# maniacs-ops/ringpop-go

Hardware: AMD Instinct MI355X
Metric: simulated member-rounds/sec at 64k members (higher is better)
Workload: dtype u32; 1 GPU; config3_cascade: 65536 members, 655 killed at r=10; rounds 5-592 timed (steady state, kill, suspect wave; faulty wave from r>=35 in window); members=65536, live_member_rounds=38153303, parallelism=1 GPU

## Files before the change

ringpop-go_amd/csrc/swimsim_engine.hip:

```cpp
#include "swimsim_kernels.hip"
#include "swimsim_xchg.hip"
#include "swimsim_census.hip"
#include "swimsim_route.hip"
#include "swimsim_forward.hip"
#include "swimsim_ringcs.hip"

#include <hipcub/hipcub.hpp>
#include <rccl/rccl.h>

#include <algorithm>
#include <cmath>
#include <condition_variable>
#include <cstdarg>
#include <cstdio>
#include <cstring>
#include <memory>
#include <mutex>
#include <string>
#include <thread>
#include <vector>

#include "../../include/swimsim.h"

using namespace swimdev;
// ... 305 lines not shown
    std::vector<hipEvent_t> round_ev;
    std::vector<float> round_ms;
    std::vector<uint32_t> wslot_h;
    std::vector<uint8_t> wused;
    std::vector<uint32_t> wcs;
    std::vector<uint32_t> wcs_ev;
    std::vector<uint4 *> wev_h;
    std::vector<unsigned long long *> wevt_h;
    uint4 *wout = nullptr;
    uint32_t *winfo = nullptr;
    uint32_t *cn_slab = nullptr, *cn_part = nullptr, *cn_nlp = nullptr, *cn_ticket = nullptr, *cn_cols = nullptr,
             *cn_res = nullptr;
    size_t cn_cap = 0;
    hipEvent_t cn_ev[2] = {nullptr, nullptr};
    uint32_t *tr_cols = nullptr, *tr_buf = nullptr, *tr_part = nullptr, *tr_nlp = nullptr, *tr_state = nullptr;
    uint32_t tr_n = 0, tr_cap = 0;
    size_t tr_bytes[5] = {0, 0, 0, 0, 0};
    struct RouteTable {
        uint32_t R;
        uint32_t *hm;
        unsigned long long *pts;
    };
    std::vector<RouteTable> rt_tabs;
    uint8_t *rt_bytes = nullptr;
    uint64_t *rt_off = nullptr;
    uint32_t *rt_kh = nullptr, *rt_p0 = nullptr, *rt_rows = nullptr, *rt_cnt = nullptr;
    int32_t *rt_base = nullptr, *rt_own = nullptr;
    uint32_t *rt_srv = nullptr;
    int32_t *rt_nbase = nullptr;
    size_t rt_srv_cap = 0, rt_nbase_cap = 0;
    unsigned long long *rt_exc = nullptr, *rt_exc2 = nullptr, *rt_uniq = nullptr, *rt_cur = nullptr;
    void *rt_cub = nullptr;
    size_t rt_bytes_cap = 0, rt_keys_cap = 0, rt_rows_cap = 0, rt_own_cap = 0, rt_exc_cap = 0, rt_cub_bytes = 0;
    std::vector<uint64_t> rt_rel;
    hipEvent_t rt_ev[2] = {nullptr, nullptr};
    unsigned long long *rc_key = nullptr;
    uint32_t *rc_cnt = nullptr, *rc_rep = nullptr, *rc_dif = nullptr, *rc_hl = nullptr, *rc_csr = nullptr, *rc_out = nullptr;
    size_t rc_cap = 0;
    bool rc_lds = false;
    double rc_split[3] = {0, 0, 0};
    int32_t *fw_own = nullptr, *fw_handler = nullptr, *fw_holder = nullptr, *fw_next = nullptr;
    uint32_t *fw_ent = nullptr, *fw_key = nullptr, *fw_bins = nullptr;
    uint8_t *fw_outcome = nullptr, *fw_hops = nullptr;
    size_t fw_own_cap = 0, fw_req_cap = 0, fw_ent_cap = 0, fw_bins_cap = 0;
    double fw_split[3] = {0, 0, 0};
    int csr_mode = 1;
    CsrSet csr, csr2;
    size_t csr_sbw_words = 0;
    uint32_t csr_ecap = 4096, csr_rcap = 1024, csr_KP = 0;
    uint64_t csr_launches = 0;
    uint32_t csr_side_min = 4097;
    int fault_inject = 0;
    int defer_test = 0;
    int cs_defer = 1;
    uint32_t rounds_left = 0;
    uint32_t round_deferred = 0;
    bool cs_carried = false;
    int resp_echo = 1;
    bool cs_defer_log = false;
    uint64_t cs_skipped_rounds = 0, cs_carried_rows = 0, cs_forced = 0, cs_units_base[3] = {0, 0, 0};
    bool colx_stale = false;
    std::string err;

    int fail(int code, const char *fmt, ...) {
        char buf[512];
        va_list ap;
        va_start(ap, fmt);
        vsnprintf(buf, sizeof buf, fmt, ap);
        va_end(ap);
        err = buf;
        return code;
    }
};

#define HIPCHK(h, x)                                                                             \
    do {                                                                                         \
        hipError_t e_ = (x);                                                                     \
        if (e_ != hipSuccess) return (h)->fail(SWIMSIM_EHIP, "%s: %s", #x, hipGetErrorString(e_)); \
    } while (0)

namespace {

template <typename T>
int dalloc(swimsim *h, T **p, size_t count, const char *what) {
    void *q = nullptr;
    size_t bytes = std::max<size_t>(count * sizeof(T), 16);
    hipError_t e = hipMalloc(&q, bytes);
    if (e != hipSuccess) return h->fail(SWIMSIM_ENOMEM, "hipMalloc(%s, %zu bytes): %s", what, bytes, hipGetErrorString(e));
    h->allocs.push_back(q);
    h->alloc_bytes += bytes;
    *p = (T *)q;
    return 0;
}

template <typename T>
void dfree(swimsim *h, T **p, size_t bytes) {
    if (!*p) return;
    auto it = std::find(h->allocs.begin(), h->allocs.end(), (void *)*p);
    if (it != h->allocs.end()) h->allocs.erase(it);
    hipFree(*p);
    h->alloc_bytes -= bytes;
    *p = nullptr;
}

hipEvent_t take_event(swimsim *h) {
    if (!h->evpool.empty()) {
        hipEvent_t e = h->evpool.back();
        h->evpool.pop_back();
        return e;
    }
    hipEvent_t e;
    hipEventCreate(&e);
    return e;
}

struct Scope {
    swimsim *h;
    int fam;
    hipStream_t st;
    hipEvent_t a{}, b{};
    bool on;
    Scope(swimsim *h_, int f, hipStream_t st_ = nullptr)
        : h(h_), fam(f), st(st_ ? st_ : h_->s), on(h_->timing && ((h_->timing_mask >> f) & 1u)) {
        if (on) {
            a = take_event(h);
            hipEventRecord(a, st);
        }
    }
    ~Scope() {
        if (on) {
            b = take_event(h);
            hipEventRecord(b, st);
            h->pending.push_back(Timed{fam, a, b});
        }
    }
};

void drain_timing(swimsim *h) {
    if (h->pending.empty()) return;
    hipStreamSynchronize(h->s);
    for (auto &t : h->pending) {
        float ms = 0;
        hipEventElapsedTime(&ms, t.a, t.b);
        h->fam_ms[t.fam] += ms;
        h->fam_n[t.fam]++;
        h->evpool.push_back(t.a);
        h->evpool.push_back(t.b);
    }
    h->pending.clear();
}

constexpr uint32_t SWIM_WAVE_BLOCK = 256;
constexpr uint32_t kWavesPerBlock = SWIM_WAVE_BLOCK / 64;
inline uint32_t blocks_for_waves(uint32_t waves) { return waves ? (waves + kWavesPerBlock - 1) / kWavesPerBlock : 1; }
inline uint32_t blocks_for_threads(uint32_t n) { return n ? (n + 255) / 256 : 1; }
inline uint32_t rep_slots(uint32_t nl) { uint32_t s = 1024; while (s < 2 * nl) s <<= 1; return s; }

constexpr uint32_t kMaxEcap = 1u << 24;

int build_tail_table(swimsim *h, uint32_t ecap) {
    if (ecap > kMaxEcap)
        return h->fail(SWIMSIM_ERANGE, "incarnation step %u beyond the checksum tables (at most 2^24 steps of the period)",
                       ecap - 1);
    std::vector<uint32_t> t((size_t)ecap * 4 * 8, 0u);
    uint32_t max_tl = 0, min_tl = 0xFFFFFFFFu;
    for (uint32_t e = 0; e < ecap; e++) {
        char digits[32];
        snprintf(digits, sizeof digits, "%lld", (long long)(h->t0 + (int64_t)e * h->period));
        for (uint32_t s = 0; s < 4; s++) {
            char buf[64];
            int n = snprintf(buf, sizeof buf, "%s%s;", kStatus[s], digits);
            if (n > 24) return h->fail(SWIMSIM_EINVAL, "incarnation %s too long for the checksum tail table", digits);
            uint8_t bytes[24] = {0};
            memcpy(bytes, buf, (size_t)n);
            uint32_t *dst = &t[((size_t)e * 4 + s) * 8];
            for (int w = 0; w < 6; w++)
                dst[w] = (uint32_t)bytes[4 * w] | ((uint32_t)bytes[4 * w + 1] << 8) | ((uint32_t)bytes[4 * w + 2] << 16) |
                         ((uint32_t)bytes[4 * w + 3] << 24);
            dst[6] = (uint32_t)n;
            max_tl = std::max(max_tl, (uint32_t)n);
            min_tl = std::min(min_tl, (uint32_t)n);
        }
    }
    std::vector<uint32_t> rt((size_t)ecap * 4 * 8, 0u);
    const uint32_t q = h->W / 4, r = h->W % 4;
    for (size_t i = 0; i < (size_t)ecap * 4; i++) {
        uint8_t bytes[32] = {0};
        const uint32_t n = t[i * 8 + 6];
        memcpy(bytes + r, &t[i * 8], n);
        for (int w = 0; w < 7; w++)
            rt[i * 8 + w] = (uint32_t)bytes[4 * w] | ((uint32_t)bytes[4 * w + 1] << 8) | ((uint32_t)bytes[4 * w + 2] << 16) |
                            ((uint32_t)bytes[4 * w + 3] << 24);
        const uint32_t L = h->W + n;
        const uint8_t *tb = (const uint8_t *)&t[i * 8];
        rt[i * 8 + 7] = (uint32_t)tb[n - 4] | ((uint32_t)tb[n - 3] << 8) | ((uint32_t)tb[n - 2] << 16) |
                        ((uint32_t)tb[n - 1] << 24);
        if (r + n > 27) return h->fail(SWIMSIM_EINVAL, "record tail too long for the checksum tail table");
        rt[i * 8 + 6] |= L << 24;
    }
    (void)q;
    std::vector<uint32_t> rt8((size_t)ecap * 8 * 8, 0u);
    for (size_t e = 0; e < ecap; e++)
        for (int s = 0; s < 4; s++) memcpy(&rt8[(e * 8 + s) * 8], &rt[(e * 4 + s) * 8], 32);
    uint32_t *dev = nullptr, *rdev = nullptr, *r8dev = nullptr;
    if (int rc = dalloc(h, &dev, t.size(), "tail table")) return rc;
    if (int rc = dalloc(h, &rdev, rt.size(), "record tail table")) return rc;
    if (int rc = dalloc(h, &r8dev, rt8.size(), "record tail table by member word")) return rc;
    HIPCHK(h, hipMemcpy(dev, t.data(), t.size() * 4, hipMemcpyHostToDevice));
    HIPCHK(h, hipMemcpy(rdev, rt.data(), rt.size() * 4, hipMemcpyHostToDevice));
    HIPCHK(h, hipMemcpy(r8dev, rt8.data(), rt8.size() * 4, hipMemcpyHostToDevice));
    h->d.tailw = dev;
    h->d.rtail = rdev;
    h->d.rtail8 = r8dev;
    {
        uint32_t d0 = t[6] - 6, nthr = 0;
        for (int k = 0; k < 8; k++) h->d.dig_thr[k] = 0xFFFFFFFFu;
        uint32_t prev = d0;
        for (uint32_t e = 1; e < ecap; e++) {
            const uint32_t de = t[((size_t)e * 4) * 8 + 6] - 6;
            if (de != prev) {
                if (de != prev + 1 || nthr == 8) return h->fail(SWIMSIM_EINVAL, "incarnation digit count changes too often");
                h->d.dig_thr[nthr++] = e;
                prev = de;
            }
        }
        h->d.dig_d0 = d0;
    }
    h->ecap = ecap;
    h->d.ecap = ecap;
    h->max_tl = max_tl;
    h->d.max_tail = max_tl;
    h->d.min_tail = min_tl;
    h->fast_cs = (h->W == 19 && h->W + max_tl <= 40);
    return 0;
}

hipError_t stream_sync(swimsim *h) {
    if (!h->sync_spin || !h->ev_rt) return hipStreamSynchronize(h->s);
    const hipError_t prior = hipPeekAtLastError();
    hipError_t e = hipEventRecord(h->ev_rt, h->s);
    if (e != hipSuccess) return e;
    while ((e = hipEventQuery(h->ev_rt)) == hipErrorNotReady) {
    }
    (void)hipGetLastError();
    return prior != hipSuccess ? prior : e;
}

int check_err(swimsim *h) {
    uint32_t e = 0;
    HIPCHK(h, hipMemcpyAsync(&e, h->d.err, 4, hipMemcpyDeviceToHost, h->s));
    HIPCHK(h, stream_sync(h));
    if (!e) return 0;
    hipMemsetAsync(h->d.err, 0, 4, h->s);
    if (e & E_POOL) return h->fail(SWIMSIM_ECAPACITY, "message pool overflow (raise message_pool_bytes)");
    if (e & E_DENSE) return h->fail(SWIMSIM_ECAPACITY, "dense snapshot pool overflow");
    if (e & E_ECAP) return h->fail(SWIMSIM_ECAPACITY, "incarnation beyond the checksum table");
    if (e & E_SHORT) return h->fail(SWIMSIM_EINVAL, "checksum string of <= 24 bytes is not supported");
    if (e & E_ITER) return h->fail(SWIMSIM_EINVAL, "iterator found no pingable member despite a positive count");
    return h->fail(SWIMSIM_EINVAL, "dissemination count mismatch (internal error %u)", e);
}

int read_counters(swimsim *h, uint64_t *out ) {
    std::vector<uint64_t> c((size_t)CTR_SHARDS * CTR_STRIDE);
    HIPCHK(h, hipMemcpyAsync(c.data(), h->d.ctr, c.size() * 8, hipMemcpyDeviceToHost, h->s));
    HIPCHK(h, stream_sync(h));
    for (int i = 0; i < CTR_STRIDE; i++) {
        uint64_t t = 0;
        for (int k = 0; k < CTR_SHARDS; k++) t += c[(size_t)k * CTR_STRIDE + i];
        out[i] = t;
    }
    return 0;
}

int build_inbox(swimsim *h, uint32_t nlocal, uint32_t n) {
    Scope sc(h, F_SORT);
    h->inbox_n = n;
    if (n > nlocal)
        hipLaunchKernelGGL(k_inbox_count, dim3(blocks_for_threads(n - nlocal)), dim3(256), 0, h->s, h->d, h->keys, nlocal,
                           n, h->counts, h->kslot);
    h->scan_gen = h->scan_gen % 0x1FFFFFu + 1u;
    hipLaunchKernelGGL(k_inbox_scan, dim3((h->NL + 1023) / 1024), dim3(1024), 0, h->s, h->d, h->counts, h->offs,
                       h->ulist, h->scan_agg, h->scan_gen);
    hipLaunchKernelGGL(k_inbox_place, dim3(blocks_for_threads(n)), dim3(256), 0, h->s, h->d, h->keys, n, h->offs,
                       h->kslot, h->vals_in, h->run_of);
    return 0;
}

inline uint32_t owner_host(const swimsim *h, uint32_t o) {
    uint32_t r = 0;
    while (r + 1 < h->G && o >= h->shard_lo[r + 1]) r++;
    return r;
}

XArgs xargs(swimsim *h) {
    XArgs x{};
    x.sdesc = h->sdesc; x.sdesc2 = h->sdesc2; x.rdesc = h->rdesc; x.rdesc2 = h->rdesc2; x.snapdesc = h->snapdesc;
    x.hdesc = h->hdesc;
    x.sI = h->sI; x.sC = h->sC; x.sI2 = h->sI2; x.sC2 = h->sC2;
    x.hsics = h->hsics;
    x.need = h->need;
    x.keys = h->keys; x.npairs = h->npairs; x.keycap = h->keycap;
    x.needlist = h->needlist; x.needcnt = h->needcnt; x.needcap = h->needcap;
    x.sS = h->sS; x.sS2 = h->sS2; x.rcs = h->rcs;
    x.csreq = h->csreq; x.csreqcnt = h->csreqcnt; x.csreqcap = h->keycap;
    return x;
}
// ... 2414 lines not shown
```

ringpop-go_amd/csrc/swimsim_kernels.hip:

```cpp
#include "swimsim_kernels.h"

namespace swimdev {

#define SWIM_DPP(old, src, ctrl, rm) ((uint32_t)__builtin_amdgcn_update_dpp((int)(old), (int)(src), (ctrl), (rm), 0xf, false))
template <typename Op>
__device__ __forceinline__ uint32_t dpp_scan(uint32_t x, uint32_t id, Op op) {
    x = op(x, SWIM_DPP(id, x, 0x111, 0xf));
    x = op(x, SWIM_DPP(id, x, 0x112, 0xf));
    x = op(x, SWIM_DPP(id, x, 0x114, 0xf));
    x = op(x, SWIM_DPP(id, x, 0x118, 0xf));
    x = op(x, SWIM_DPP(id, x, 0x142, 0xa));
    x = op(x, SWIM_DPP(id, x, 0x143, 0xc));
    return x;
}
__device__ __forceinline__ uint32_t dpp_scan_add(uint32_t x) { return dpp_scan(x, 0u, [](uint32_t a, uint32_t b) { return a + b; }); }
__device__ __forceinline__ uint32_t dpp_scan_umin(uint32_t x) {
    return dpp_scan(x, 0xFFFFFFFFu, [](uint32_t a, uint32_t b) { return min(a, b); });
}
__device__ __forceinline__ int32_t dpp_scan_imax(int32_t x) {
    return (int32_t)dpp_scan((uint32_t)x, 0x80000000u, [](uint32_t a, uint32_t b) { return (uint32_t)max((int32_t)a, (int32_t)b); });
}
__device__ __forceinline__ int32_t dpp_scan_imin(int32_t x) {
    return (int32_t)dpp_scan((uint32_t)x, 0x7FFFFFFFu, [](uint32_t a, uint32_t b) { return (uint32_t)min((int32_t)a, (int32_t)b); });
}
// ... 864 lines not shown
__global__ void k_nhe_reset(DS d) {
    const uint32_t ol = blockIdx.x * blockDim.x + threadIdx.x;
    if (ol < d.NL) d.nhe[ol] = d.dcnt[ol];
}

__global__ void __launch_bounds__(1024) k_hot_extend(DS d) {
    __shared__ uint32_t n;
    if (threadIdx.x == 0) {
        n = d.hot_cnt[0];
        d.hot_cnt[1] = n;
    }
    __syncthreads();
    for (uint32_t w = threadIdx.x; w < d.NBIT; w += blockDim.x) {
        uint32_t bits = d.hotnew[w];
        if (!bits) continue;
        d.hotnew[w] = 0;
        while (bits) {
            const uint32_t m = w * 32 + (uint32_t)(__ffs(bits) - 1);
            bits &= bits - 1;
            if (m >= d.N || d.hidx[m] != SRC_NONE) continue;
            const uint32_t k = atomicAdd(&n, 1u);
            if (k < d.HP) {
                d.hidx[m] = k;
                d.hlist[k] = m;
            }
        }
    }
    __syncthreads();
    if (threadIdx.x == 0) d.hot_cnt[0] = min(n, d.HP);
}

__global__ void k_hot_fill(DS d) {
    const uint32_t ol = wave_gid();
    if (ol >= d.NL) return;
    const uint32_t k0 = d.hot_cnt[1], k1 = d.hot_cnt[0];
    const size_t rb = (size_t)ol * d.NP, hb = (size_t)ol * d.HP;
    int nowhot = 0;
    for (uint32_t k = k0 + lane_id(); k < k1; k += 64 * MB) {
        uint32_t m[MB], w[MB];
        uint2 cell[MB];
#pragma unroll
        for (int u = 0; u < MB; u++) m[u] = k + 64u * u < k1 ? d.hlist[k + 64u * u] : 0u;
#pragma unroll
        for (int u = 0; u < MB; u++) {
            cell[u] = d.dent[rb + m[u]];
            w[u] = d.mw[rb + m[u]];
        }
#pragma unroll
        for (int u = 0; u < MB; u++) {
            if (k + 64u * u >= k1) continue;
            d.hmw[hb + k + 64u * u] = w[u];
            d.hde[hb + k + 64u * u] = cell[u];
            nowhot += de_p(cell[u].x) != DP_NONE;
        }
    }
    if (k1 > k0) {
        nowhot = wsum(nowhot);
        if (lane_id() == 0 && nowhot) d.nhe[ol] -= nowhot;
    }
}

__global__ void k_hot_flush(DS d, uint32_t ol0, uint32_t nrows) {
    const uint32_t i = wave_gid();
    if (i >= nrows) return;
    const uint32_t ol = ol0 + i, k1 = d.hot_cnt[0];
    const size_t rb = (size_t)ol * d.NP, hb = (size_t)ol * d.HP;
    for (uint32_t k = lane_id(); k < k1; k += 64) d.dent[rb + d.hlist[k]] = d.hde[hb + k];
}

__global__ void k_add_join_list(DS d, uint32_t ol, const uint4 *__restrict__ rec, uint32_t n, uint32_t r,
                                uint32_t *applied_out) {
    const uint32_t o = d.lo + ol;
    const uint32_t now = wave_clock(d, o, r);
    const uint32_t *rowp = d.mw + (size_t)ol * d.NP;
    MAcc acc;
    acc_begin(d, ol, acc);
    for (uint32_t base = 0; base < n; base += 64 * MB) {
        uint4 c[MB];
        uint32_t cur[MB];
#pragma unroll
        for (int u = 0; u < MB; u++) {
            const uint32_t i = base + u * 64 + lane_id();
            c[u] = i < n ? rec[i] : make_uint4(0xFFFFFFFFu, 0, 0, 0);
        }
#pragma unroll
        for (int u = 0; u < MB; u++) cur[u] = c[u].x != 0xFFFFFFFFu ? rowp[c[u].x & 0xFFFFFFu] : 0u;
#pragma unroll
        for (int u = 0; u < MB; u++) {
            if (c[u].x == 0xFFFFFFFFu) continue;
            const uint32_t m = c[u].x & 0xFFFFFFu;
            const int before = acc.napp;
            merge_change_w(d, ol, o, m, cur[u], c[u].x >> 24, c[u].y, c[u].z, c[u].w, now, now, acc);
            if (acc.napp != before && m != o) {
                const size_t idx = (size_t)ol * d.NP + m;
                d.dent[idx].x = DE_NONE;
                const uint32_t hk = hot_slot(d, m);
                if (hk != SRC_NONE) d.hde[(size_t)ol * d.HP + hk].x = DE_NONE;
                else acc.dnh--;
                atomicAnd(&d.dbit[(size_t)ol * d.NBIT + (m >> 5)], ~(1u << (m & 31)));
                acc.ddc--;
            }
        }
    }
    const int napp = wsum(acc.napp);
    __threadfence_block();
    wave_finalize(d, ol, acc, 2);
    if (lane_id() == 0) *applied_out = (uint32_t)napp;
}

__device__ int thread_make_change(const DS &d, uint32_t ol, uint32_t o, uint32_t m, uint32_t e, uint32_t st, uint32_t now) {
    MAcc acc;
    acc_begin(d, ol, acc);
    const uint32_t self_e = d.mw[(size_t)ol * d.NP + o] >> 3;
    merge_change(d, ol, o, m, st, e, o, self_e, now, now, acc);
    fold_row(d, ol, acc.dping, acc.ddc, acc.napp, acc.nref, 0, acc.dlen, acc.maxlast, acc.inval, acc.dfp, true, acc.dnh);
    return acc.napp;
}

__global__ void k_events(DS d, const uint4 *ev, uint32_t nev, uint32_t r, uint32_t *applied_out) {
    if (threadIdx.x != 0 || blockIdx.x != 0) return;
    for (uint32_t i = 0; i < nev; i++) {
        const uint4 e = ev[i];
        const uint32_t kind = e.x, o = e.y;
        if (kind == 5) {
            d.coff[o] = (int32_t)e.w;
            if (applied_out) applied_out[i] = 0;
            continue;
        }
        if (o < d.lo || o >= d.lo + d.NL) continue;
        const uint32_t ol = o - d.lo;
        const uint32_t now = clock_of(d, o, r);
        int applied = 0;
        switch (kind) {
        case 1:
            applied = thread_make_change(d, ol, o, e.z, e.w & 0x1FFFFFFFu, e.w >> 29, now);
            break;
        case 2:
            applied = thread_make_change(d, ol, o, o, now, ST_ALIVE, now);
            break;
        case 3:
            applied = thread_make_change(d, ol, o, o, d.mw[(size_t)ol * d.NP + o] >> 3, ST_LEAVE, now);
            break;
        case 4:
            for (uint32_t m = 0; m < d.N; m++) {
                const uint32_t w = d.mw[(size_t)ol * d.NP + m];
                if ((w & 7u) == ST_FAULTY) applied += thread_make_change(d, ol, o, m, w >> 3, ST_TOMB, now);
            }
            break;
        }
        if (applied_out) applied_out[i] = (uint32_t)applied;
    }
}

__global__ void k_timers(DS d, uint32_t round) {
    const uint32_t ol = wave_gid();
    if (ol >= d.NL) return;
    const uint32_t o = d.lo + ol;
    const uint32_t r = wave_clock(d, o, round);
    if (!d.live[o] || d.tmin[ol] > r) return;
    const uint32_t self_e = d.mw[(size_t)ol * d.NP + o] >> 3;
    MAcc acc;
    const unsigned long long tbase = d.useq ? d.useq[ol] : 0ull;
    uint32_t newmin = NO_DEADLINE;
    int fired = 0;
    for (uint32_t b0 = 0; b0 < d.NB; b0 += 64) {
        const uint32_t bl = b0 + lane_id();
        const uint32_t bm = bl < d.NB ? d.tblk[(size_t)ol * d.NB + bl] : NO_DEADLINE;
        unsigned long long due = __ballot(bm <= r);
        if (bm > r) newmin = min(newmin, bm);
        while (due) {
            const uint32_t bb = __ffsll((long long)due) - 1;
            due &= due - 1;
            const uint32_t b = b0 + bb;
            const uint32_t m = (b << 6) + lane_id();
            const size_t idx = (size_t)ol * d.NP + m;
            const uint8_t ts = d.tst[idx];
            const uint32_t state = ts & 7u;
            uint2 a = d.tmr[idx];
            if (state && !(ts & 0x80) && a.x <= r) {
                d.tst[idx] = ts | 0x80;
                fired++;
                acc.tag = tbase + ((0xFFFFull - min(r - a.x, 0xFFFFu)) << 24) + m;
                if (state == ST_SUSPECT) merge_change(d, ol, o, m, ST_FAULTY, a.y, o, self_e, r, a.x, acc);
                else if (state == ST_FAULTY) merge_change(d, ol, o, m, ST_TOMB, a.y, o, self_e, r, a.x, acc);
                else {
                    const uint32_t w = d.mw[idx];
                    if ((w & 7u) != ST_UNKNOWN && m != o) {
                        if (is_pingable(w & 7u)) acc.dping--;
                        d.mw[idx] = (w & ~7u) | ST_UNKNOWN;
                        colmark(d, m);
                        const uint32_t hk = hot_slot(d, m);
                        if (hk != SRC_NONE) d.hmw[(size_t)ol * d.HP + hk] = (w & ~7u) | ST_UNKNOWN;
                        track_len(d, ol, m, w, (w & ~7u) | ST_UNKNOWN, acc);
                        acc.dfp += fpmix(m, (w & ~7u) | ST_UNKNOWN) - fpmix(m, w);
                        acc.evict++;
                    }
                }
                a = d.tmr[idx];
            }
            const uint8_t ts2 = d.tst[idx];
            const uint32_t v = ((ts2 & 7u) && !(ts2 & 0x80)) ? a.x : NO_DEADLINE;
            const uint32_t bmin = wmin(v);
            if (lane_id() == 0) d.tblk[(size_t)ol * d.NB + b] = bmin;
            newmin = min(newmin, bmin);
        }
    }
    newmin = wmin(newmin);
    if (lane_id() == 0) d.tmin[ol] = newmin;
    fired = wsum(fired);
    if (lane_id() == 0 && fired) ctr_add(d, C_TIMERS_FIRED, (unsigned long long)fired);
    const int napp_t = wsum(acc.napp);
    if (lane_id() == 0 && napp_t && d.useq) d.useq[ol] = tbase + (1ull << 40);
    __threadfence_block();
    wave_finalize(d, ol, acc, 0, false);
}

__global__ void k_select(DS d, int32_t *tgt, uint32_t *exh_list, uint32_t *exh_cnt, uint32_t *counts, uint32_t *info) {
    const uint32_t ol = blockIdx.x * blockDim.x + threadIdx.x;
    if (ol == 0) { info[2] = 0u; *d.dense_cur = 0u; }
    if (ol >= d.NL) return;
    counts[ol] = 0u;
    const uint32_t o = d.lo + ol;
    int32_t target = -1;
    if (d.live[o]) {
        if (d.ping[ol] <= 0) {
            exh_list[atomicAdd(exh_cnt, 1u)] = ol;
        } else {
            int32_t idx = d.it_idx[ol];
            uint32_t ep = d.it_ep[ol];
            Feistel f;
            f.init(d.seed, o, ep, d.N);
            const uint32_t *row = d.mw + (size_t)ol * d.NP;
            for (uint32_t guard = 0; guard < 4 * d.N + 8; guard++) {
                idx++;
                if (idx >= (int32_t)d.N) { idx = 0; ep++; f.init(d.seed, o, ep, d.N); }
                const uint32_t m = f.perm((uint32_t)idx, d.N);
                const uint32_t st = row[m] & 7u;
                if (st == ST_UNKNOWN) continue;
                if (m != o && is_pingable(st)) { target = (int32_t)m; break; }
            }
            if (target < 0) atomicOr(d.err, E_ITER);
            d.it_idx[ol] = idx;
            d.it_ep[ol] = ep;
        }
    }
    tgt[ol] = target;
}

__global__ void k_select_exhaust(DS d, const uint32_t *exh_list, const uint32_t *exh_cnt, uint32_t *scratch) {
    const uint32_t cnt = *exh_cnt;
    uint32_t *vis = scratch + (size_t)blockIdx.x * (d.NP / 32);
    for (uint32_t q = blockIdx.x; q < cnt; q += gridDim.x) {
        const uint32_t ol = exh_list[q], o = d.lo + ol;
        for (uint32_t i = threadIdx.x; i < d.NP / 32; i += blockDim.x) vis[i] = 0;
        __syncthreads();
        if (threadIdx.x == 0) {
            const uint32_t *row = d.mw + (size_t)ol * d.NP;
            uint32_t known = 0;
            for (uint32_t m = 0; m < d.N; m++) known += (row[m] & 7u) != ST_UNKNOWN;
            int32_t idx = d.it_idx[ol];
            uint32_t ep = d.it_ep[ol], nvis = 0;
            Feistel f;
            f.init(d.seed, o, ep, d.N);
            uint64_t guard = 0;
            while (nvis < known && guard++ < 8ull * d.N + 8) {
                idx++;
                if (idx >= (int32_t)d.N) { idx = 0; ep++; f.init(d.seed, o, ep, d.N); }
                const uint32_t m = f.perm((uint32_t)idx, d.N);
                if ((row[m] & 7u) == ST_UNKNOWN) continue;
                if (!(vis[m >> 5] & (1u << (m & 31)))) { vis[m >> 5] |= 1u << (m & 31); nvis++; }
            }
            d.it_idx[ol] = idx;
            d.it_ep[ol] = ep;
        }
        __syncthreads();
    }
}

__global__ void k_list(DS d, int mode, const int32_t *tgt, const uint8_t *failed, uint32_t *list, uint32_t *cnt) {
    const uint32_t ol = blockIdx.x * blockDim.x + threadIdx.x;
    if (ol >= d.NL) return;
    const uint32_t dv = d.dirty[ol];
    bool take = dv != 0;
    if (mode == 1) take = take && tgt[ol] >= 0;
    if (mode == 2) take = take && failed[ol];
    if (take) list[atomicAdd(cnt, 1u)] = ol;
    if (take && mode == 0) d.cpslot[ol] = SRC_NONE;
    if (mode == 0) {
        const unsigned long long fresh = __ballot(dv == 1u);
        if (fresh && lane_id() == 0) atomicAdd(cnt + 1, (uint32_t)__popcll(fresh));
    }
}

__global__ void k_carry(DS d) {
    const uint32_t ol = blockIdx.x * blockDim.x + threadIdx.x;
    if (ol < d.NL && d.dirty[ol]) d.dirty[ol] = DIRTY_CARRIED;
}

__global__ void k_list_one(uint32_t *list, uint32_t *cnt, uint32_t ol, const DS d) {
    if (threadIdx.x == 0) { *cnt = d.dirty[ol] ? 1u : 0u; list[0] = ol; }
}

__global__ void k_issue(DS d, int mode, const int32_t *tgt, const uint8_t *failed, MsgDesc *sdesc, uint32_t *sI,
                        uint32_t *sC, uint32_t *sS) {
    const uint32_t ol = wave_gid();
    if (ol >= d.NL) return;
    const uint32_t o = d.lo + ol;
    if ((mode == 0 && tgt[ol] < 0) || (mode == 1 && !failed[ol])) {
        if (sS && lane_id() == 0) sS[o] = SRC_NONE;
        return;
    }
    const uint32_t dirty = d.dirty[ol], cpslot = d.cpslot[ol], cs = d.cs[ol], selfw = d.mw[(size_t)ol * d.NP + o];
    const uint32_t clen = d.clen[ol];
    const int32_t clast = d.clast[ol];
    MsgDesc md;
    wave_issue(d, ol, md);
    uint32_t slot = SRC_NONE;
    if (sS && dirty && !d.ulog) {
        MsgDesc sn;
        if (wave_snapshot(d, ol, o, sn)) slot = sn.off_lo;
        if (lane_id() == 0) ctr_add(d, C_X_ISSUE_SNAPS, 1ull);
    } else if (sS && dirty) {
        slot = SRC_PEND;
        if (lane_id() == 0) { d.ilen[ol] = clen; d.ilast[ol] = clast; }
    } else if (sS) {
        slot = cpslot;
    }
    if (lane_id() == 0) {
        sdesc[o] = md;
        sI[o] = selfw >> 3;
        sC[o] = slot == SRC_NONE ? cs : 0u;
        if (sS) sS[o] = slot;
        if (mode == 0) {
            ctr_add(d, C_PINGS, 1ull);
            ctr_add(d, C_MSG_CHANGES, (unsigned long long)md.len);
        }
        ctr_add(d, C_X_ISSUED, (unsigned long long)md.len);
    }
}

__device__ __forceinline__ void inbox_count(const DS &d, unsigned long long key, uint32_t *counts, uint32_t *kslot,
                                            uint32_t i) {
    const uint32_t u = (uint32_t)(key >> 32) - d.lo;
    if (u < d.NL) kslot[i] = atomicAdd(&counts[u], 1u);
}

__device__ __forceinline__ void x_push(uint4 *items, uint32_t *cnt, uint32_t cap, uint32_t *err, uint4 it) {
    const uint32_t i = atomicAdd(cnt, 1u);
    if (i < cap) items[i] = it;
    else atomicOr(err, E_XCAP);
}

__global__ void k_pairs_direct(DS d, const int32_t *tgt, unsigned long long *keys, uint8_t *failed, uint32_t *info,
                               uint4 *xitems, uint32_t *xcnt, uint32_t xcap, uint32_t *counts, uint32_t *kslot) {
    const uint32_t ol = blockIdx.x * blockDim.x + threadIdx.x;
    if (ol >= d.NL) return;
    const uint32_t o = d.lo + ol;
    const int32_t t = tgt[ol];
    unsigned long long key = (unsigned long long)d.N << 32;
// ... 1010 lines not shown
```

Baseline: 126.3 million member-rounds/s.

## Batch due timers into per-wave LDS queues and prefetch timer blocks ahead

k_timers now scans due timer blocks in groups of eight, prefetching block minima and state bytes ahead. Due entries are compacted into a per-wave LDS ring queue and fired 64 at a time, so every lane does useful work instead of one divergent lane per block. This targets low lane utilisation and serial memory latency during the suspect and faulty waves. It adds LDS use, register pressure, a merge_change_w variant and a manual waitcnt, and the ring ordering and tblk minimum recomputation must match the old semantics.

Measured after the change: 128.5 million member-rounds/s, median of 6. 1.02x the previous value.

```diff
diff --git a/ringpop-go_amd/csrc/swimsim_engine.hip b/ringpop-go_amd/csrc/swimsim_engine.hip
--- a/ringpop-go_amd/csrc/swimsim_engine.hip
+++ b/ringpop-go_amd/csrc/swimsim_engine.hip
@@ -481,6 +481,7 @@
 
 constexpr uint32_t SWIM_WAVE_BLOCK = 256;
 constexpr uint32_t kWavesPerBlock = SWIM_WAVE_BLOCK / 64;
+static_assert(kWavesPerBlock == swimdev::TIMER_WAVES, "k_timers has one LDS queue per wave of its workgroup");
 inline uint32_t blocks_for_waves(uint32_t waves) { return waves ? (waves + kWavesPerBlock - 1) / kWavesPerBlock : 1; }
 inline uint32_t blocks_for_threads(uint32_t n) { return n ? (n + 255) / 256 : 1; }
 inline uint32_t rep_slots(uint32_t nl) { uint32_t s = 1024; while (s < 2 * nl) s <<= 1; return s; }
diff --git a/ringpop-go_amd/csrc/swimsim_kernels.hip b/ringpop-go_amd/csrc/swimsim_kernels.hip
--- a/ringpop-go_amd/csrc/swimsim_kernels.hip
+++ b/ringpop-go_amd/csrc/swimsim_kernels.hip
@@ -1040,7 +1040,14 @@
     }
 }
 
-__global__ void k_timers(DS d, uint32_t round) {
+constexpr int TG = 8;
+constexpr uint32_t TQ = 128;
+static_assert((TQ & (TQ - 1)) == 0 && TQ >= 128, "the queue is a ring that holds 64 waiting entries and 64 new ones");
+constexpr uint32_t TIMER_WAVES = 4;
+constexpr int WAITCNT_VM0 = 0x0F70;
+__global__ void __launch_bounds__(64 * TIMER_WAVES) k_timers(DS d, uint32_t round) {
+    __shared__ uint32_t q_m[TIMER_WAVES][TQ];
+    __shared__ uint2 q_a[TIMER_WAVES][TQ];
     const uint32_t ol = wave_gid();
     if (ol >= d.NL) return;
     const uint32_t o = d.lo + ol;
@@ -1051,48 +1058,134 @@
     const unsigned long long tbase = d.useq ? d.useq[ol] : 0ull;
     uint32_t newmin = NO_DEADLINE;
     int fired = 0;
-    for (uint32_t b0 = 0; b0 < d.NB; b0 += 64) {
-        const uint32_t bl = b0 + lane_id();
-        const uint32_t bm = bl < d.NB ? d.tblk[(size_t)ol * d.NB + bl] : NO_DEADLINE;
-        unsigned long long due = __ballot(bm <= r);
-        if (bm > r) newmin = min(newmin, bm);
-        while (due) {
-            const uint32_t bb = __ffsll((long long)due) - 1;
-            due &= due - 1;
-            const uint32_t b = b0 + bb;
-            const uint32_t m = (b << 6) + lane_id();
+    uint32_t *qm = q_m[(threadIdx.x >> 6) & (TIMER_WAVES - 1u)];
+    uint2 *qa = q_a[(threadIdx.x >> 6) & (TIMER_WAVES - 1u)];
+    uint32_t qh = 0, qn = 0;
+    auto fire = [&](uint32_t n) {
+        __threadfence_block();
+        __builtin_amdgcn_s_waitcnt(WAITCNT_VM0);
+        const bool on = lane_id() < n;
+        const uint32_t qi = (qh + lane_id()) & (TQ - 1u);
+        const uint32_t pm = on ? qm[qi] : 0u;
+        const uint2 a = on ? qa[qi] : make_uint2(0u, 0u);
+        qh = (qh + n) & (TQ - 1u);
+        qn -= n;
+        if (on) {
+            const uint32_t m = pm & 0xFFFFFFu, state = pm >> 24;
             const size_t idx = (size_t)ol * d.NP + m;
-            const uint8_t ts = d.tst[idx];
-            const uint32_t state = ts & 7u;
-            uint2 a = d.tmr[idx];
-            if (state && !(ts & 0x80) && a.x <= r) {
-                d.tst[idx] = ts | 0x80;
-                fired++;
-                acc.tag = tbase + ((0xFFFFull - min(r - a.x, 0xFFFFu)) << 24) + m;
-                if (state == ST_SUSPECT) merge_change(d, ol, o, m, ST_FAULTY, a.y, o, self_e, r, a.x, acc);
-                else if (state == ST_FAULTY) merge_change(d, ol, o, m, ST_TOMB, a.y, o, self_e, r, a.x, acc);
-                else {
-                    const uint32_t w = d.mw[idx];
-                    if ((w & 7u) != ST_UNKNOWN && m != o) {
-                        if (is_pingable(w & 7u)) acc.dping--;
-                        d.mw[idx] = (w & ~7u) | ST_UNKNOWN;
-                        colmark(d, m);
-                        const uint32_t hk = hot_slot(d, m);
-                        if (hk != SRC_NONE) d.hmw[(size_t)ol * d.HP + hk] = (w & ~7u) | ST_UNKNOWN;
-                        track_len(d, ol, m, w, (w & ~7u) | ST_UNKNOWN, acc);
-                        acc.dfp += fpmix(m, (w & ~7u) | ST_UNKNOWN) - fpmix(m, w);
-                        acc.evict++;
-                    }
-                }
-                a = d.tmr[idx];
+            const uint32_t cur = d.mw[idx];
+            const uint32_t hk = hot_slot(d, m);
+            d.tst[idx] = (uint8_t)(state | 0x80u);
+            fired++;
+            acc.tag = tbase + ((0xFFFFull - min(r - a.x, 0xFFFFu)) << 24) + m;
+            if (state == ST_SUSPECT || state == ST_FAULTY) {
+                merge_change_w(d, ol, o, m, cur, state == ST_SUSPECT ? ST_FAULTY : ST_TOMB, a.y, o, self_e, r, a.x, acc, hk);
+            } else if ((cur & 7u) != ST_UNKNOWN && m != o) {
+                const uint32_t w = cur;
+                if (is_pingable(w & 7u)) acc.dping--;
+                d.mw[idx] = (w & ~7u) | ST_UNKNOWN;
+                colmark(d, m);
+                if (hk != SRC_NONE) d.hmw[(size_t)ol * d.HP + hk] = (w & ~7u) | ST_UNKNOWN;
+                track_len(d, ol, m, w, (w & ~7u) | ST_UNKNOWN, acc);
+                acc.dfp += fpmix(m, (w & ~7u) | ST_UNKNOWN) - fpmix(m, w);
+                acc.evict++;
             }
             const uint8_t ts2 = d.tst[idx];
-            const uint32_t v = ((ts2 & 7u) && !(ts2 & 0x80)) ? a.x : NO_DEADLINE;
-            const uint32_t bmin = wmin(v);
-            if (lane_id() == 0) d.tblk[(size_t)ol * d.NB + b] = bmin;
+            if ((ts2 & 7u) && !(ts2 & 0x80)) newmin = min(newmin, d.tmr[idx].x);
+        }
+    };
+    uint32_t *brow = d.tblk + (size_t)ol * d.NB;
+    const uint8_t *srow = d.tst + (size_t)ol * d.NP;
+    const uint2 *trow = d.tmr + (size_t)ol * d.NP;
+    uint32_t b0 = 0, bnext = 0;
+    unsigned long long due = 0;
+    uint32_t bm_next = lane_id() < d.NB ? brow[lane_id()] : NO_DEADLINE;
+    uint32_t bm_next2 = 64u + lane_id() < d.NB ? brow[64u + lane_id()] : NO_DEADLINE;
+    auto next_block = [&]() -> uint32_t {
+        while (!due) {
+            if (bnext >= d.NB) return SRC_NONE;
+            const uint32_t bm = bm_next;
+            b0 = bnext;
+            bnext += 64u;
+            const uint32_t bl = bnext + 64u + lane_id();
+            bm_next = bm_next2;
+            bm_next2 = bl < d.NB ? brow[bl] : NO_DEADLINE;
+            due = __ballot(bm <= r);
+            if (bm > r) newmin = min(newmin, bm);
+        }
+        const uint32_t b = b0 + (uint32_t)__ffsll((long long)due) - 1u;
+        due &= due - 1;
+        return b;
+    };
+    auto append = [&](uint32_t m, uint32_t tsu, uint2 au, bool isdue, unsigned long long dmask) {
+        if (isdue) {
+            const uint32_t at = (qh + qn + (uint32_t)__popcll(dmask & lanemask_lt())) & (TQ - 1u);
+            qm[at] = m | (tsu << 24);
+            qa[at] = au;
+        }
+        qn += (uint32_t)__popcll(dmask);
+    };
+    uint32_t bbn[TG], tsn[TG];
+#pragma unroll
+    for (int u = 0; u < TG; u++) {
+        bbn[u] = next_block();
+        tsn[u] = bbn[u] != SRC_NONE ? (uint32_t)srow[(bbn[u] << 6) + lane_id()] : 0u;
+    }
+    while (bbn[0] != SRC_NONE) {
+        uint32_t bb[TG], ts[TG];
+        uint2 a[TG];
+#pragma unroll
+        for (int u = 0; u < TG; u++) { bb[u] = bbn[u]; ts[u] = tsn[u]; }
+#pragma unroll
+        for (int u = 0; u < TG; u++) {
+            bbn[u] = next_block();
+            tsn[u] = bbn[u] != SRC_NONE ? (uint32_t)srow[(bbn[u] << 6) + lane_id()] : 0u;
+        }
+#pragma unroll
+        for (int u = 0; u < TG; u++) {
+            const bool armed = (ts[u] & 7u) && !(ts[u] & 0x80u);
+            a[u] = armed ? trow[(bb[u] << 6) + lane_id()] : make_uint2(NO_DEADLINE, 0u);
+        }
+        unsigned long long dm[TG];
+        uint32_t gc = 0;
+#pragma unroll
+        for (int u = 0; u < TG; u++) {
+            const bool isdue = a[u].x <= r;
+            dm[u] = __ballot(isdue);
+            gc += (uint32_t)__popcll(dm[u]);
+            const uint32_t bmin = wmin(isdue ? NO_DEADLINE : a[u].x);
+            if (lane_id() == 0 && bb[u] != SRC_NONE) brow[bb[u]] = bmin;
             newmin = min(newmin, bmin);
         }
-    }
+        if (!gc) continue;
+        uint32_t pend = 0;
+        if (qn + gc <= TQ) {
+#pragma unroll
+            for (int u = 0; u < TG; u++)
+                if (dm[u]) append((bb[u] << 6) + lane_id(), ts[u], a[u], a[u].x <= r, dm[u]);
+        } else {
+#pragma unroll
+            for (int u = 0; u < TG; u++)
+                if (dm[u]) pend |= 1u << u;
+        }
+        do {
+            if (pend) {
+                const uint32_t u = (uint32_t)__ffs((int)pend) - 1u;
+                pend &= pend - 1u;
+                uint32_t bu = bb[0];
+#pragma unroll
+                for (int k = 1; k < TG; k++)
+                    if ((uint32_t)k == u) bu = bb[k];
+                const uint32_t m = (bu << 6) + lane_id();
+                const uint32_t tsu = srow[m];
+                const bool armed = (tsu & 7u) && !(tsu & 0x80u);
+                const uint2 au = armed ? trow[m] : make_uint2(NO_DEADLINE, 0u);
+                append(m, tsu, au, au.x <= r, __ballot(au.x <= r));
+            }
+            if (qn >= 64u) fire(64u);
+        } while (pend);
+    }
+    if (qn) fire(qn);
     newmin = wmin(newmin);
     if (lane_id() == 0) d.tmin[ol] = newmin;
     fired = wsum(fired);
```
